# hi-paris/Prosody-Control-French-TTS

Measured on AMD Instinct MI355X. Metric: audio-seconds/sec prosody+align throughput, 16 kHz French, higher is better.
Workload: dtype fp16-resid16 (MFMA legs) + f64 (F0 / LUFS)

## Files before the change

prosody-control-french-tts_amd/csrc/pce_align.hip:

```cpp
#include "pce_internal.h"
#include <vector>

namespace {

constexpr int DTW_MAXN = 1024;

__global__ __launch_bounds__(DTW_MAXN) void k_dtw(const double *__restrict__ x, int64_t x_stride, int ld, const int *__restrict__ n_rows,
                                                 const int *__restrict__ n_cols, int N_max, int M_max, unsigned char *__restrict__ trace,
                                                 int *__restrict__ path_i, int *__restrict__ path_j, int *__restrict__ path_len)
{
    __shared__ float diag[3][DTW_MAXN + 1];
    const int b = blockIdx.x, t = threadIdx.x;
    const int N = n_rows ? n_rows[b] : N_max, M = n_cols ? n_cols[b] : M_max;
    if (N <= 0 || M <= 0) { if (t == 0) path_len[b] = 0; return; }
    const double *xb = x + (size_t)b * (size_t)x_stride;
    unsigned char *tr = trace + (size_t)b * (size_t)(N_max + 1) * (size_t)(M_max + 1);
    const float INF = __builtin_huge_valf();
    for (int r = t; r <= N; r += blockDim.x) { diag[0][r] = INF; diag[1][r] = INF; diag[2][r] = INF; }
    __syncthreads();
    if (t == 0) diag[0][0] = 0.0f;
    __syncthreads();
    const int r = t + 1;
    for (int D = 2; D <= N + M; D++) {
        float *cur = diag[D % 3]; const float *p1 = diag[(D - 1) % 3], *p2 = diag[(D - 2) % 3];
        const int c = D - r;
        if (t < N && c >= 1 && c <= M) {
            const float c0 = p2[r - 1], c1 = p1[r - 1], c2 = p1[r];
            float cm; unsigned char tt;
            if (c0 < c1 && c0 < c2) { cm = c0; tt = 0; }
            else if (c1 < c0 && c1 < c2) { cm = c1; tt = 1; }
            else { cm = c2; tt = 2; }
            cur[r] = (float)(xb[(size_t)(r - 1) * ld + (c - 1)] + (double)cm);
            tr[(size_t)r * (M + 1) + c] = tt;
        } else if (t < N) {
            cur[r] = INF;
        }
        if (t == 0) cur[0] = INF;
        __syncthreads();
    }
    __threadfence_block();
    if (t == 0) {
        int i = N, j = M, n = 0;
        int *pi = path_i + (size_t)b * (N_max + M_max), *pj = path_j + (size_t)b * (N_max + M_max);
        while (i > 0 || j > 0) {
            pi[n] = i - 1; pj[n] = j - 1; n++;
            const int tt = (i == 0) ? 2 : (j == 0) ? 1 : tr[(size_t)i * (M + 1) + j];
            if (tt == 0) { i--; j--; } else if (tt == 1) { i--; } else { j--; }
        }
        for (int a = 0, z = n - 1; a < z; a++, z--) {
            const int ti = pi[a], tj = pj[a]; pi[a] = pi[z]; pj[a] = pj[z]; pi[z] = ti; pj[z] = tj;
        }
        path_len[b] = n;
    }
}

__global__ __launch_bounds__(DTW_MAXN) void k_nw(const int *__restrict__ a_ids, const long long *__restrict__ a_off, const int *__restrict__ b_ids,
                                                const long long *__restrict__ b_off, int match, int mismatch, int gap,
                                                unsigned char *__restrict__ trace, const long long *__restrict__ tr_off,
                                                int *__restrict__ out_i, int *__restrict__ out_j, const long long *__restrict__ out_off,
                                                int *__restrict__ out_len, int *__restrict__ rows, const long long *__restrict__ rows_off)
{
    __shared__ int diag[3][DTW_MAXN + 1];
    const int b = blockIdx.x, t = threadIdx.x, S = (int)blockDim.x;
    const int N = (int)(a_off[b + 1] - a_off[b]), M = (int)(b_off[b + 1] - b_off[b]);
    const int *A = a_ids + a_off[b], *B = b_ids + b_off[b];
    unsigned char *tr = trace + tr_off[b];
    int *top = rows + rows_off[b], *bot = top + (M + 1);
    for (int r0 = 0; r0 < N; r0 += S) {
        const int R = min(S, N - r0), lr = t + 1, gr = r0 + lr;
        const bool first = r0 == 0, more = r0 + S < N;
        const int my_a = t < R ? A[gr - 1] : 0;
        if (t == 0) diag[0][0] = r0 * gap;
        int tv = (t == 0 && M >= 1) ? (first ? gap : top[1]) : 0;
        __syncthreads();
        for (int D = 1; D <= R + M; D++) {
            int *cur = diag[D % 3]; const int *p1 = diag[(D + 2) % 3], *p2 = diag[(D + 1) % 3];
            const int c = D - lr;
            if (t < R) {
                if (c >= 1 && c <= M) {
                    const int dg = p2[lr - 1] + (my_a == B[c - 1] ? match : mismatch), up = p1[lr - 1] + gap, lf = p1[lr] + gap;
                    int best = dg; unsigned char tt = 0;
                    if (up > best) { best = up; tt = 1; }
                    if (lf > best) { best = lf; tt = 2; }
                    cur[lr] = best;
                    tr[(size_t)gr * (M + 1) + c] = tt;
                    if (more && lr == R) bot[c] = best;
                } else if (c == 0) {
                    cur[lr] = gr * gap;
                }
            }
            if (t == 0 && D <= M) { cur[0] = tv; if (D + 1 <= M) tv = first ? (D + 1) * gap : top[D + 1]; }
            __syncthreads();
        }
        if (more) { __threadfence(); __syncthreads(); int *x = top; top = bot; bot = x; }
    }
    __threadfence_block();
    if (t == 0) {
        int i = N, j = M, n = 0;
        int *pi = out_i + out_off[b], *pj = out_j + out_off[b];
        while (i > 0 || j > 0) {
            const int tt = (i == 0) ? 2 : (j == 0) ? 1 : tr[(size_t)i * (M + 1) + j];
            if (tt == 0) { pi[n] = i - 1; pj[n] = j - 1; i--; j--; }
            else if (tt == 1) { pi[n] = i - 1; pj[n] = -1; i--; }
            else { pi[n] = -1; pj[n] = j - 1; j--; }
            n++;
        }
        for (int x = 0, z = n - 1; x < z; x++, z--) {
            const int ti = pi[x], tj = pj[x]; pi[x] = pi[z]; pj[x] = pj[z]; pi[z] = ti; pj[z] = tj;
        }
        out_len[b] = n;
    }
}

__global__ __launch_bounds__(256) void k_levenshtein(const unsigned *__restrict__ a_chars, const long long *__restrict__ a_off,
                                                     const unsigned *__restrict__ b_chars, const long long *__restrict__ b_off, int batch,
                                                     int *__restrict__ rows, const long long *__restrict__ rows_off, int *__restrict__ out)
{
    const int lane = threadIdx.x & 63, pair = blockIdx.x * 4 + __builtin_amdgcn_readfirstlane((int)(threadIdx.x >> 6));
    if (pair >= batch) return;
    int N = (int)(a_off[pair + 1] - a_off[pair]), M = (int)(b_off[pair + 1] - b_off[pair]);
    const unsigned *A = a_chars + a_off[pair], *B = b_chars + b_off[pair];
    if (N > M) { const unsigned *t = A; A = B; B = t; const int n = N; N = M; M = n; }
    if (N == 0) { if (lane == 0) out[pair] = M; return; }
    int *top = rows + rows_off[pair], *bot = top + (M + 1);
    const int n_stripes = (N + 63) >> 6;
    for (int s = 0; s < n_stripes; s++) {
        const int r0 = s << 6, R = min(64, N - r0), last = R - 1;
        const bool more = s + 1 < n_stripes;
        const unsigned my_a = lane < R ? A[r0 + lane] : 0u;
        int cur = r0 + lane + 1;
        int up = r0 + lane;
        unsigned bch = 0u;
        unsigned chB = lane < M ? B[lane] : 0u, nxB = 0u;
        int chT = s == 0 ? lane + 1 : (lane + 1 <= M ? top[lane + 1] : 0), nxT = 0;
        int botc = r0 + R;
        const int steps = M + R - 1;
        for (int t = 0; t < steps; t++) {
            const int k = t & 63;
            if (k == 0) {
                if (t) { chB = nxB; chT = nxT; }
                const int c1 = t + 64 + lane;
                nxB = c1 < M ? B[c1] : 0u;
                nxT = s == 0 ? c1 + 1 : (c1 + 1 <= M ? top[c1 + 1] : 0);
            }
            const unsigned b_in = (unsigned)__builtin_amdgcn_readlane((int)chB, k);
            const int top_in = __builtin_amdgcn_readlane(chT, k);
            const int upn_s = __builtin_amdgcn_update_dpp(0, cur, 0x138, 0xF, 0xF, true);
            const unsigned bch_s = (unsigned)__builtin_amdgcn_update_dpp(0, (int)bch, 0x138, 0xF, 0xF, true);
            const int upn = lane == 0 ? top_in : upn_s;
            bch = lane == 0 ? b_in : bch_s;
            const int c = t - lane + 1;
            if (lane < R && c >= 1 && c <= M) {
                const int sub = up + (my_a != bch ? 1 : 0), ins = upn + 1, del = cur + 1;
                cur = min(min(ins, del), sub);
                up = upn;
            }
            if (more) {
                const int cb = t - last + 1;
                if (cb >= 1) {
                    const int v = __builtin_amdgcn_readlane(cur, last);
                    if (lane == (cb & 63)) botc = v;
                    if ((cb & 63) == 63 || cb == M) {
                        const int base = cb & ~63;
                        if (lane <= (cb & 63)) bot[base + lane] = botc;
                    }
                }
            }
        }
        if (!more) { if (lane == last) out[pair] = cur; }
        else { __threadfence(); int *x = top; top = bot; bot = x; }
    }
}

}

int pce_dtw_launch(pce_ctx *c, const double *d_x, int64_t x_stride, int ld, const int *d_rows, const int *d_cols, int N_max, int M_max,
                   int batch, unsigned char *d_trace, int *d_pi, int *d_pj, int *d_pl)
{
    if (N_max > DTW_MAXN) return pce_fail(c, PCE_E_LIMIT, "DTW supports at most %d rows", DTW_MAXN);
    KernelTimer t(c, PCE_K_DTW);
    const int threads = ((N_max + 63) / 64) * 64;
    hipLaunchKernelGGL(k_dtw, dim3((unsigned)batch), dim3((unsigned)threads), 0, c->stream, d_x, x_stride, ld, d_rows, d_cols, N_max, M_max,
                       d_trace, d_pi, d_pj, d_pl);
    PCE_HIP(c, hipGetLastError());
    return PCE_OK;
}

extern "C" {

int pce_dtw(pce_ctx *c, const double *x, int32_t n_rows, int32_t n_cols, int32_t batch, int32_t *path_i, int32_t *path_j, int32_t *path_len)
{
    if (!c || !x || !path_i || !path_j || !path_len || n_rows <= 0 || n_cols <= 0 || batch <= 0) return PCE_E_INVALID;
    PCE_HIP(c, hipSetDevice(c->device));
    const size_t cells = (size_t)batch * n_rows * n_cols, pl = (size_t)batch * (size_t)(n_rows + n_cols);
    DevBuf dx, dtr, dpi, dpj, dpl;
    PCE_UPLOAD(c, dx, x, cells);
    PCE_HIP(c, dtr.reserve((size_t)batch * (size_t)(n_rows + 1) * (size_t)(n_cols + 1)));
    PCE_HIP(c, dpi.reserve(sizeof(int) * pl)); PCE_HIP(c, dpj.reserve(sizeof(int) * pl)); PCE_HIP(c, dpl.reserve(sizeof(int) * (size_t)batch));
    PCE_TRY(pce_dtw_launch(c, dx.as<double>(), (int64_t)n_rows * n_cols, n_cols, nullptr, nullptr, n_rows, n_cols, batch,
                           dtr.as<unsigned char>(), dpi.as<int>(), dpj.as<int>(), dpl.as<int>()));
    PCE_FETCH(c, path_i, dpi.p, pl);
    PCE_FETCH(c, path_j, dpj.p, pl);
    PCE_FETCH(c, path_len, dpl.p, (size_t)batch);
    PCE_HIP(c, hipStreamSynchronize(c->stream));
    pce_profile_collect(c);
    return PCE_OK;
}

int pce_nw_align(pce_ctx *c, const int32_t *a_ids, const int64_t *a_off, const int32_t *b_ids, const int64_t *b_off, int32_t batch,
                 int32_t match, int32_t mismatch, int32_t gap, int32_t *out_i, int32_t *out_j, int32_t *out_len)
{
    if (!c || !a_off || !b_off || !out_i || !out_j || !out_len || batch <= 0) return PCE_E_INVALID;
    PCE_HIP(c, hipSetDevice(c->device));
    std::vector<long long> tro((size_t)batch + 1, 0), oo((size_t)batch + 1, 0), rwo((size_t)batch + 1, 0);
    int max_rows = 0;
    for (int32_t b = 0; b < batch; b++) {
        const int64_t n = a_off[b + 1] - a_off[b], m = b_off[b + 1] - b_off[b];
        if (n < 0 || m < 0) return pce_fail(c, PCE_E_INVALID, "pce_nw_align: offsets of pair %d decrease", b);
        if (n > 0x3fffffff || m > 0x3fffffff) return pce_fail(c, PCE_E_LIMIT, "pce_nw_align: pair %d is longer than 2^30 tokens", b);
        tro[(size_t)b + 1] = tro[(size_t)b] + (n + 1) * (m + 1);
        rwo[(size_t)b + 1] = rwo[(size_t)b] + (n > DTW_MAXN ? 2 * (m + 1) : 0);
        oo[(size_t)b + 1] = oo[(size_t)b] + n + m;
        if (n > max_rows) max_rows = (int)n;
    }
    const size_t na = (size_t)a_off[batch], nb = (size_t)b_off[batch], no = (size_t)oo[(size_t)batch];
    if (a_off[0] != 0 || b_off[0] != 0) return pce_fail(c, PCE_E_INVALID, "pce_nw_align: offsets must start at 0");
    if ((na && !a_ids) || (nb && !b_ids)) return PCE_E_INVALID;
    DevBuf da, db, dao, dbo, dtr, dtro, doi, doj, doo, dol, drw, drwo;
    PCE_HIP(c, drw.reserve(sizeof(int) * ((size_t)rwo[(size_t)batch] + 1))); PCE_HIP(c, dtr.reserve((size_t)tro[(size_t)batch] + 1));
    PCE_HIP(c, doi.reserve(sizeof(int) * (no + 1))); PCE_HIP(c, doj.reserve(sizeof(int) * (no + 1))); PCE_HIP(c, dol.reserve(sizeof(int) * (size_t)batch));
    PCE_UPLOAD(c, da, a_ids, na, 1); PCE_UPLOAD(c, db, b_ids, nb, 1);
    PCE_UPLOAD(c, dao, a_off, (size_t)batch + 1); PCE_UPLOAD(c, dbo, b_off, (size_t)batch + 1);
    PCE_UPLOAD(c, dtro, tro); PCE_UPLOAD(c, doo, oo); PCE_UPLOAD(c, drwo, rwo);
    int threads = 64; while (threads < max_rows && threads < DTW_MAXN) threads <<= 1;
    {
        KernelTimer t(c, PCE_K_NW);
        hipLaunchKernelGGL(k_nw, dim3((unsigned)batch), dim3((unsigned)threads), 0, c->stream, da.as<int>(), dao.as<long long>(), db.as<int>(),
                           dbo.as<long long>(), match, mismatch, gap, dtr.as<unsigned char>(), dtro.as<long long>(), doi.as<int>(), doj.as<int>(),
                           doo.as<long long>(), dol.as<int>(), drw.as<int>(), drwo.as<long long>());
    }
    PCE_HIP(c, hipGetLastError());
    if (no) {
        PCE_FETCH(c, out_i, doi.p, no);
        PCE_FETCH(c, out_j, doj.p, no);
    }
    PCE_FETCH(c, out_len, dol.p, (size_t)batch);
    PCE_HIP(c, hipStreamSynchronize(c->stream));
    pce_profile_collect(c);
    return PCE_OK;
}

int pce_levenshtein(pce_ctx *c, const uint32_t *a_chars, const int64_t *a_off, const uint32_t *b_chars, const int64_t *b_off, int32_t batch,
                    int32_t *out_dist)
{
    if (!c || !a_off || !b_off || !out_dist || batch <= 0) return PCE_E_INVALID;
    PCE_HIP(c, hipSetDevice(c->device));
    if (a_off[0] != 0 || b_off[0] != 0) return pce_fail(c, PCE_E_INVALID, "pce_levenshtein: offsets must start at 0");
    std::vector<long long> ro((size_t)batch + 1, 0);
    for (int32_t b = 0; b < batch; b++) {
        const int64_t n = a_off[b + 1] - a_off[b], m = b_off[b + 1] - b_off[b];
        if (n < 0 || m < 0) return pce_fail(c, PCE_E_INVALID, "pce_levenshtein: offsets of pair %d decrease", b);
        if (n > 0x3fffffff || m > 0x3fffffff) return pce_fail(c, PCE_E_LIMIT, "pce_levenshtein: pair %d is longer than 2^30 characters", b);
        const int64_t shorter = n < m ? n : m, longer = n < m ? m : n;
        ro[(size_t)b + 1] = ro[(size_t)b] + (shorter > 64 ? 2 * (longer + 1) : 0);
    }
    const size_t na = (size_t)a_off[batch], nb = (size_t)b_off[batch];
    if ((na && !a_chars) || (nb && !b_chars)) return PCE_E_INVALID;
    DevBuf da, db, dao, dbo, dro, drows, dout;
    PCE_HIP(c, drows.reserve(sizeof(int) * ((size_t)ro[(size_t)batch] + 1))); PCE_HIP(c, dout.reserve(sizeof(int) * (size_t)batch));
    PCE_UPLOAD(c, da, a_chars, na, 1); PCE_UPLOAD(c, db, b_chars, nb, 1);
    PCE_UPLOAD(c, dao, a_off, (size_t)batch + 1); PCE_UPLOAD(c, dbo, b_off, (size_t)batch + 1); PCE_UPLOAD(c, dro, ro);
    {
        KernelTimer t(c, PCE_K_LEVENSHTEIN);
        hipLaunchKernelGGL(k_levenshtein, dim3((unsigned)((batch + 3) / 4)), dim3(256), 0, c->stream, da.as<unsigned>(), dao.as<long long>(),
                           db.as<unsigned>(), dbo.as<long long>(), batch, drows.as<int>(), dro.as<long long>(), dout.as<int>());
    }
    PCE_HIP(c, hipGetLastError());
    PCE_FETCH(c, out_dist, dout.p, (size_t)batch);
    PCE_HIP(c, hipStreamSynchronize(c->stream));
    pce_profile_collect(c);
    return PCE_OK;
}

}
```

prosody-control-french-tts_amd/csrc/pce_attention.inc:

```
constexpr int AT_QB = 128;

struct AttnArgs {
    const op_t *q; int64_t q_ld;
    const op_t *k; int64_t k_ld;
    const op_t *vt; int64_t vt_clip; int vt_sp;
    const int *q_row0, *q_len, *k_row0, *k_len;
    op_t *out; int64_t out_ld;
    int causal;
    int *fell_back;
};

template <bool EXACT, bool NT>
__device__ __forceinline__ bool attn_block16(const AttnArgs &A, op_t *smem, int bx, int head, int clip)
{
    constexpr int NS = 3, DPW = 4;
    const int tid = threadIdx.x, lane = tid & 63, wv = __builtin_amdgcn_readfirstlane(tid >> 6);
    const int n16 = lane & 15, g = lane >> 4;
    const int Sq = A.q_len[clip], Sk = A.k_len[clip];
    const int q0 = bx * AT_QB + wv * 32;
    const op_t *qbase = A.q + (int64_t)A.q_row0[clip] * A.q_ld + head * 64;
    const op_t *kbase = A.k + (int64_t)A.k_row0[clip] * A.k_ld + head * 64;
    const op_t *vtbase = A.vt + (int64_t)clip * A.vt_clip + (int64_t)head * 64 * A.vt_sp;
    const int kld = (int)A.k_ld, vsp = A.vt_sp;
    const __amdgpu_buffer_rsrc_t rsK = __builtin_amdgcn_make_buffer_rsrc(const_cast<op_t *>(kbase), 0, ((Sk - 1) * kld + 64) * 2, 0x00020000);
    const __amdgpu_buffer_rsrc_t rsV = __builtin_amdgcn_make_buffer_rsrc(const_cast<op_t *>(vtbase), 0, 64 * vsp * 2, 0x00020000);
    int voffK[2], voffV[2];
#pragma unroll
    for (int i = 0; i < 2; i++) {
        const int row = (wv + 4 * i) * 8 + (lane >> 3), c8 = swz_chunk(row, lane & 7) * 8;
        const int kb = row >> 4, rho = row & 15;
        const int key = 32 * (kb >> 1) + 8 * (rho >> 2) + 4 * (kb & 1) + (rho & 3);
        voffK[i] = (key * kld + c8) * 2; voffV[i] = (row * vsp + c8) * 2;
    }
    auto stage = [&](int t) {
        op_t *sK = smem + (t % NS) * (2 * 64 * 64), *sV = sK + 64 * 64;
        const int key0 = t * 64;
#pragma unroll
        for (int i = 0; i < 2; i++) {
            __builtin_amdgcn_raw_ptr_buffer_load_lds(rsK, (__attribute__((address_space(3))) void *)(sK + (wv + 4 * i) * 8 * 64), 16, voffK[i], key0 * kld * 2, 0, NT ? 3 : 0);
            __builtin_amdgcn_raw_ptr_buffer_load_lds(rsV, (__attribute__((address_space(3))) void *)(sV + (wv + 4 * i) * 8 * 64), 16, voffV[i], key0 * 2, 0, NT ? 3 : 0);
        }
    };
    const f32x4 z4 = {0.f, 0.f, 0.f, 0.f};
    opx8 qf[2][2];
    int my_q[2];
#pragma unroll
    for (int qb = 0; qb < 2; qb++) {
        my_q[qb] = q0 + 16 * qb + n16;
        int qr = my_q[qb]; if (qr >= Sq) qr = Sq - 1;
        const op_t *qp = qbase + (int64_t)qr * A.q_ld;
#pragma unroll
        for (int ks = 0; ks < 2; ks++) qf[qb][ks] = *reinterpret_cast<const opx8 *>(qp + 32 * ks + 8 * g);
    }
    opx8 ones;
#pragma unroll
    for (int j = 0; j < 8; j++) ones[j] = (op_t)(n16 == 0 ? 1.0f : 0.0f);
    f32x4 o[4][2], osum[2];
#pragma unroll
    for (int db = 0; db < 4; db++) { o[db][0] = z4; o[db][1] = z4; }
    osum[0] = z4; osum[1] = z4;
    float m_run[2] = {-1e30f, -1e30f}, l_run[2] = {0.f, 0.f};
    const float sl2 = 0.125f * 1.4426950408889634f;
    int k_need = Sk;
    if (A.causal) k_need = min(Sk, bx * AT_QB + AT_QB);
    const int nt = (k_need + 63) / 64;
    int kaddr[4][2], vaddr[4][2];
#pragma unroll
    for (int b4 = 0; b4 < 4; b4++)
#pragma unroll
        for (int ks = 0; ks < 2; ks++) {
            const int row = 16 * b4 + n16;
            kaddr[b4][ks] = row * 64 + swz_chunk(row, 4 * ks + g) * 8;
            vaddr[b4][ks] = 64 * 64 + row * 64 + swz_chunk(row, 4 * ks + g) * 8;
        }
    stage(0);
    if (nt > 1) stage(1);
    for (int kt = 0; kt < nt; kt++) {
        if (kt + 1 < nt) __builtin_amdgcn_s_waitcnt(0x0F70 | DPW); else __builtin_amdgcn_s_waitcnt(0x0F70 | 0);
        __builtin_amdgcn_s_barrier();
        if (kt + 2 < nt) stage(kt + 2);
        const op_t *sC = smem + (kt % NS) * (2 * 64 * 64);
        f32x4 sc[4][2];
#pragma unroll
        for (int kb = 0; kb < 4; kb++)
#pragma unroll
            for (int ks = 0; ks < 2; ks++) {
                const opx8 kf = *reinterpret_cast<const opx8 *>(&sC[kaddr[kb][ks]]);
#pragma unroll
                for (int qb = 0; qb < 2; qb++) sc[kb][qb] = mfma16(kf, qf[qb][ks], ks == 0 ? z4 : sc[kb][qb]);
            }
        if ((kt * 64 + 63 >= Sk) || (A.causal && kt * 64 + 63 > q0)) {
#pragma unroll
            for (int kb = 0; kb < 4; kb++)
#pragma unroll
                for (int i = 0; i < 4; i++) {
                    const int key = kt * 64 + 32 * (kb >> 1) + 8 * g + 4 * (kb & 1) + i;
#pragma unroll
                    for (int qb = 0; qb < 2; qb++) {
                        const bool vis = key < Sk && (!A.causal || key <= my_q[qb]);
                        sc[kb][qb][i] = vis ? sc[kb][qb][i] : -1e30f;
                    }
                }
        }
        if (EXACT || kt == 0) {
            float mx[2];
#pragma unroll
            for (int qb = 0; qb < 2; qb++) {
                float m = sc[0][qb][0];
#pragma unroll
                for (int kb = 0; kb < 4; kb++)
#pragma unroll
                    for (int i = 0; i < 4; i++) m = fmaxf(m, sc[kb][qb][i]);
                m = m > -1e29f ? m * sl2 : -1e30f;
                m = fmaxf(m, __shfl_xor(m, 16, 64));
                m = fmaxf(m, __shfl_xor(m, 32, 64));
                mx[qb] = fmaxf(m_run[qb], m);
            }
            if (__builtin_amdgcn_ballot_w64(mx[0] > m_run[0] || mx[1] > m_run[1]) != 0) {
#pragma unroll
                for (int qb = 0; qb < 2; qb++) {
                    const float corr = __builtin_amdgcn_exp2f(m_run[qb] - mx[qb]);
                    l_run[qb] *= corr;
#pragma unroll
                    for (int db = 0; db < 4; db++)
#pragma unroll
                        for (int i = 0; i < 4; i++) o[db][qb][i] *= corr;
                    m_run[qb] = mx[qb];
                }
            }
            if (!EXACT && std::is_same<op_t, _Float16>::value) { m_run[0] += 4.0f; m_run[1] += 4.0f; }
        }
        float rs[2] = {0.f, 0.f};
#pragma unroll
        for (int kb = 0; kb < 4; kb++)
#pragma unroll
            for (int qb = 0; qb < 2; qb++)
#pragma unroll
                for (int i = 0; i < 4; i++) {
                    const float pv = __builtin_amdgcn_exp2f(fmaf(sc[kb][qb][i], sl2, -m_run[qb]));
                    sc[kb][qb][i] = pv;
                    if (EXACT) rs[qb] += pv;
                }
        if (EXACT) {
#pragma unroll
            for (int qb = 0; qb < 2; qb++) {
                float sum = rs[qb];
                sum += __shfl_xor(sum, 16, 64);
                sum += __shfl_xor(sum, 32, 64);
                l_run[qb] += sum;
            }
        }
        opx8 vf[4][2];
#pragma unroll
        for (int db = 0; db < 4; db++)
#pragma unroll
            for (int s2 = 0; s2 < 2; s2++) vf[db][s2] = *reinterpret_cast<const opx8 *>(&sC[vaddr[db][s2]]);
#pragma unroll
        for (int s2 = 0; s2 < 2; s2++)
#pragma unroll
            for (int qb = 0; qb < 2; qb++) {
                opx8 pf;
#pragma unroll
                for (int i = 0; i < 4; i++) { pf[i] = (op_t)sc[2 * s2][qb][i]; pf[4 + i] = (op_t)sc[2 * s2 + 1][qb][i]; }
#pragma unroll
                for (int db = 0; db < 4; db++) o[db][qb] = mfma16(vf[db][s2], pf, o[db][qb]);
                if (!EXACT) osum[qb] = mfma16(ones, pf, osum[qb]);
            }
    }
    if (!EXACT) {
        l_run[0] = __shfl(osum[0][0], n16, 64);
        l_run[1] = __shfl(osum[1][0], n16, 64);
    }
    const bool ok = EXACT || (((l_run[0] > 0.f && l_run[0] < 1.0e30f) || my_q[0] >= Sq) && ((l_run[1] > 0.f && l_run[1] < 1.0e30f) || my_q[1] >= Sq));
    if (!EXACT && __syncthreads_or(!ok)) return false;
    typedef __attribute__((ext_vector_type(4))) op_t opx4;
#pragma unroll
    for (int qb = 0; qb < 2; qb++) {
        if (my_q[qb] >= Sq) continue;
        const float inv = 1.0f / l_run[qb];
        op_t *op = A.out + ((int64_t)A.q_row0[clip] + my_q[qb]) * A.out_ld + head * 64;
#pragma unroll
        for (int db = 0; db < 4; db++) {
            opx4 v4;
#pragma unroll
            for (int i = 0; i < 4; i++) v4[i] = (op_t)(o[db][qb][i] * inv);
            *reinterpret_cast<opx4 *>(op + 16 * db + 4 * g) = v4;
        }
    }
    return true;
}

template <bool NT>
__global__ __launch_bounds__(256, 3) void k_attention_lean16(AttnArgs A, int force_exact )
{
    __shared__ __attribute__((aligned(1024))) op_t smem[3 * 2 * 64 * 64];
    const unsigned nx = gridDim.x, ny = gridDim.y, total = nx * ny * gridDim.z;
    const unsigned lin = blockIdx.x + nx * (blockIdx.y + ny * blockIdx.z), xcd = lin & 7u, per = total >> 3, rem = total & 7u;
    const unsigned logical = xcd * per + (xcd < rem ? xcd : rem) + (lin >> 3);
    const int bx = (int)(logical % nx), head = (int)((logical / nx) % ny), clip = (int)(logical / (nx * ny));
    if (bx * AT_QB >= A.q_len[clip]) return;
    if (!force_exact && attn_block16<false, NT>(A, smem, bx, head, clip)) return;
    if (!force_exact && A.fell_back && threadIdx.x == 0) atomicAdd(A.fell_back, 1);
    __syncthreads();
    attn_block16<true, NT>(A, smem, bx, head, clip);
}

static void launch_attention(pce_ctx *c, dim3 grid, const AttnArgs &a, double flops = 0.0, int force_exact = 0 )
{
    KernelTimer kt(c, PCE_K_ATTENTION_LEAN, nullptr, flops);
    if (grid.x == 1) hipLaunchKernelGGL(k_attention_lean16<true>, grid, dim3(256), 0, c->stream, a, force_exact);
    else hipLaunchKernelGGL(k_attention_lean16<false>, grid, dim3(256), 0, c->stream, a, force_exact);
}
static void launch_attention_rows(pce_ctx *c, int n, int H, int q_rows, const op_t *q, int64_t q_ld, const op_t *k, int64_t k_ld, const op_t *vt, int vt_sp,
                                  const int *q_row0, const int *q_len, const int *k_row0, const int *k_len, op_t *out, int causal, double flops = 0.0)
{
    AttnArgs a{};
    a.q = q; a.q_ld = q_ld; a.k = k; a.k_ld = k_ld; a.vt = vt; a.vt_clip = (int64_t)H * 64 * vt_sp; a.vt_sp = vt_sp;
    a.q_row0 = q_row0; a.q_len = q_len; a.k_row0 = k_row0; a.k_len = k_len; a.out = out; a.out_ld = H * 64; a.causal = causal;
    launch_attention(c, dim3((unsigned)div_up(q_rows, AT_QB), (unsigned)H, (unsigned)n), a, flops);
}
```

Before: 21140.

## Keep small DTW traceback in LDS, prefetch cost rows, and skip empty attention query blocks

The DTW kernel now stores the traceback matrix in shared memory when it fits, prefetches cost values in register blocks of 16 diagonals, swaps diagonal pointers instead of using modulo indexing, and uses an LDS-only barrier. Backtracking writes the path in forward order in two passes instead of reversing it afterwards. The attention kernel specialises the inner tile on how many of the wave's two 16-row query blocks are valid, skipping MFMA and softmax work for out-of-range rows, and computes K/V LDS addresses from one base to lower register pressure. These changes add register use for the prefetch buffers and code-size growth from the template instantiations.

```diff
diff --git a/prosody-control-french-tts_amd/csrc/pce_align.hip b/prosody-control-french-tts_amd/csrc/pce_align.hip
--- a/prosody-control-french-tts_amd/csrc/pce_align.hip
+++ b/prosody-control-french-tts_amd/csrc/pce_align.hip
@@ -4,44 +4,87 @@
 namespace {
 
 constexpr int DTW_MAXN = 1024;
+constexpr int DTW_LDS_TRACE = 32 * 1024;
+constexpr int DTW_XB = 16;
+
+__device__ __forceinline__ void lds_barrier()
+{
+    __builtin_amdgcn_fence(__ATOMIC_RELEASE, "workgroup", "local");
+    __builtin_amdgcn_s_barrier();
+    __builtin_amdgcn_fence(__ATOMIC_ACQUIRE, "workgroup", "local");
+}
 
 __global__ __launch_bounds__(DTW_MAXN) void k_dtw(const double *__restrict__ x, int64_t x_stride, int ld, const int *__restrict__ n_rows,
                                                  const int *__restrict__ n_cols, int N_max, int M_max, unsigned char *__restrict__ trace,
                                                  int *__restrict__ path_i, int *__restrict__ path_j, int *__restrict__ path_len)
 {
     __shared__ float diag[3][DTW_MAXN + 1];
+    __shared__ unsigned char ltr[DTW_LDS_TRACE];
     const int b = blockIdx.x, t = threadIdx.x;
     const int N = n_rows ? n_rows[b] : N_max, M = n_cols ? n_cols[b] : M_max;
     if (N <= 0 || M <= 0) { if (t == 0) path_len[b] = 0; return; }
     const double *xb = x + (size_t)b * (size_t)x_stride;
     unsigned char *tr = trace + (size_t)b * (size_t)(N_max + 1) * (size_t)(M_max + 1);
+    const bool in_lds = (int64_t)(N + 1) * (int64_t)(M + 1) <= DTW_LDS_TRACE;
     const float INF = __builtin_huge_valf();
     for (int r = t; r <= N; r += blockDim.x) { diag[0][r] = INF; diag[1][r] = INF; diag[2][r] = INF; }
     __syncthreads();
     if (t == 0) diag[0][0] = 0.0f;
     __syncthreads();
     const int r = t + 1;
-    for (int D = 2; D <= N + M; D++) {
-        float *cur = diag[D % 3]; const float *p1 = diag[(D - 1) % 3], *p2 = diag[(D - 2) % 3];
-        const int c = D - r;
-        if (t < N && c >= 1 && c <= M) {
-            const float c0 = p2[r - 1], c1 = p1[r - 1], c2 = p1[r];
-            float cm; unsigned char tt;
-            if (c0 < c1 && c0 < c2) { cm = c0; tt = 0; }
-            else if (c1 < c0 && c1 < c2) { cm = c1; tt = 1; }
-            else { cm = c2; tt = 2; }
-            cur[r] = (float)(xb[(size_t)(r - 1) * ld + (c - 1)] + (double)cm);
-            tr[(size_t)r * (M + 1) + c] = tt;
-        } else if (t < N) {
-            cur[r] = INF;
-        }
-        if (t == 0) cur[0] = INF;
-        __syncthreads();
-    }
-    __threadfence_block();
+    const double *xrow = xb + (size_t)min(t, N - 1) * ld;
+    float *cur = diag[2], *p1 = diag[1], *p2 = diag[0];
+    auto fetch = [&](double (&dst)[DTW_XB], int D0) __attribute__((always_inline)) {
+#pragma unroll
+        for (int j = 0; j < DTW_XB; j++) dst[j] = xrow[min(max(D0 + j - r - 1, 0), M - 1)];
+    };
+    auto block = [&](const double (&xc)[DTW_XB], double (&xn)[DTW_XB], int D0) __attribute__((always_inline)) {
+        fetch(xn, D0 + DTW_XB);
+#pragma unroll
+        for (int j = 0; j < DTW_XB; j++) {
+            const int D = D0 + j;
+            if (D > N + M) break;
+            const int c = D - r;
+            if (t < N && c >= 1 && c <= M) {
+                const float c0 = p2[r - 1], c1 = p1[r - 1], c2 = p1[r];
+                float cm; unsigned char tt;
+                if (c0 < c1 && c0 < c2) { cm = c0; tt = 0; }
+                else if (c1 < c0 && c1 < c2) { cm = c1; tt = 1; }
+                else { cm = c2; tt = 2; }
+                cur[r] = (float)(xc[j] + (double)cm);
+                if (in_lds) ltr[r * (M + 1) + c] = tt; else tr[(size_t)r * (M + 1) + c] = tt;
+            } else if (t < N) {
+                cur[r] = INF;
+            }
+            if (t == 0) cur[0] = INF;
+            lds_barrier();
+            float *const old = p2; p2 = p1; p1 = cur; cur = old;
+        }
+    };
+    double xa[DTW_XB], xz[DTW_XB];
+    fetch(xa, 2);
+    for (int D0 = 2; D0 <= N + M; D0 += 2 * DTW_XB) {
+        block(xa, xz, D0);
+        block(xz, xa, D0 + DTW_XB);
+    }
+    __syncthreads();
     if (t == 0) {
+        int *pi = path_i + (size_t)b * (N_max + M_max), *pj = path_j + (size_t)b * (N_max + M_max);
+        if (in_lds) {
+            int n = 0;
+            for (int i = N, j = M; i > 0 || j > 0; n++) {
+                const int tt = (i == 0) ? 2 : (j == 0) ? 1 : ltr[i * (M + 1) + j];
+                if (tt == 0) { i--; j--; } else if (tt == 1) { i--; } else { j--; }
+            }
+            path_len[b] = n;
+            for (int i = N, j = M, k = n - 1; i > 0 || j > 0; k--) {
+                pi[k] = i - 1; pj[k] = j - 1;
+                const int tt = (i == 0) ? 2 : (j == 0) ? 1 : ltr[i * (M + 1) + j];
+                if (tt == 0) { i--; j--; } else if (tt == 1) { i--; } else { j--; }
+            }
+            return;
+        }
         int i = N, j = M, n = 0;
-        int *pi = path_i + (size_t)b * (N_max + M_max), *pj = path_j + (size_t)b * (N_max + M_max);
         while (i > 0 || j > 0) {
             pi[n] = i - 1; pj[n] = j - 1; n++;
             const int tt = (i == 0) ? 2 : (j == 0) ? 1 : tr[(size_t)i * (M + 1) + j];
diff --git a/prosody-control-french-tts_amd/csrc/pce_attention.inc b/prosody-control-french-tts_amd/csrc/pce_attention.inc
--- a/prosody-control-french-tts_amd/csrc/pce_attention.inc
+++ b/prosody-control-french-tts_amd/csrc/pce_attention.inc
@@ -64,30 +64,26 @@
     int k_need = Sk;
     if (A.causal) k_need = min(Sk, bx * AT_QB + AT_QB);
     const int nt = (k_need + 63) / 64;
-    int kaddr[4][2], vaddr[4][2];
-#pragma unroll
-    for (int b4 = 0; b4 < 4; b4++)
-#pragma unroll
-        for (int ks = 0; ks < 2; ks++) {
-            const int row = 16 * b4 + n16;
-            kaddr[b4][ks] = row * 64 + swz_chunk(row, 4 * ks + g) * 8;
-            vaddr[b4][ks] = 64 * 64 + row * 64 + swz_chunk(row, 4 * ks + g) * 8;
-        }
-    stage(0);
-    if (nt > 1) stage(1);
-    for (int kt = 0; kt < nt; kt++) {
-        if (kt + 1 < nt) __builtin_amdgcn_s_waitcnt(0x0F70 | DPW); else __builtin_amdgcn_s_waitcnt(0x0F70 | 0);
-        __builtin_amdgcn_s_barrier();
-        if (kt + 2 < nt) stage(kt + 2);
+    int faddr[2];
+#pragma unroll
+    for (int ks = 0; ks < 2; ks++) {
+        faddr[ks] = n16 * 64 + swz_chunk(n16, 4 * ks + g) * 8;
+        asm volatile("" : "+v"(faddr[ks]));
+    }
+    auto kaddr = [&](int b4, int ks) __attribute__((always_inline)) { return faddr[ks] + 16 * 64 * b4; };
+    auto vaddr = [&](int b4, int ks) __attribute__((always_inline)) { return faddr[ks] + 64 * 64 + 16 * 64 * b4; };
+    const int nq = __builtin_amdgcn_readfirstlane(q0 >= Sq ? 0 : q0 + 16 >= Sq ? 1 : 2);
+    auto tile = [&](auto nq_c, int kt) __attribute__((always_inline)) {
+        constexpr int NQ = decltype(nq_c)::value;
         const op_t *sC = smem + (kt % NS) * (2 * 64 * 64);
         f32x4 sc[4][2];
 #pragma unroll
         for (int kb = 0; kb < 4; kb++)
 #pragma unroll
             for (int ks = 0; ks < 2; ks++) {
-                const opx8 kf = *reinterpret_cast<const opx8 *>(&sC[kaddr[kb][ks]]);
-#pragma unroll
-                for (int qb = 0; qb < 2; qb++) sc[kb][qb] = mfma16(kf, qf[qb][ks], ks == 0 ? z4 : sc[kb][qb]);
+                const opx8 kf = *reinterpret_cast<const opx8 *>(&sC[kaddr(kb, ks)]);
+#pragma unroll
+                for (int qb = 0; qb < NQ; qb++) sc[kb][qb] = mfma16(kf, qf[qb][ks], ks == 0 ? z4 : sc[kb][qb]);
             }
         if ((kt * 64 + 63 >= Sk) || (A.causal && kt * 64 + 63 > q0)) {
 #pragma unroll
@@ -96,7 +92,7 @@
                 for (int i = 0; i < 4; i++) {
                     const int key = kt * 64 + 32 * (kb >> 1) + 8 * g + 4 * (kb & 1) + i;
 #pragma unroll
-                    for (int qb = 0; qb < 2; qb++) {
+                    for (int qb = 0; qb < NQ; qb++) {
                         const bool vis = key < Sk && (!A.causal || key <= my_q[qb]);
                         sc[kb][qb][i] = vis ? sc[kb][qb][i] : -1e30f;
                     }
@@ -105,7 +101,7 @@
         if (EXACT || kt == 0) {
             float mx[2];
 #pragma unroll
-            for (int qb = 0; qb < 2; qb++) {
+            for (int qb = 0; qb < NQ; qb++) {
                 float m = sc[0][qb][0];
 #pragma unroll
                 for (int kb = 0; kb < 4; kb++)
@@ -116,9 +112,9 @@
                 m = fmaxf(m, __shfl_xor(m, 32, 64));
                 mx[qb] = fmaxf(m_run[qb], m);
             }
-            if (__builtin_amdgcn_ballot_w64(mx[0] > m_run[0] || mx[1] > m_run[1]) != 0) {
-#pragma unroll
-                for (int qb = 0; qb < 2; qb++) {
+            if (__builtin_amdgcn_ballot_w64(mx[0] > m_run[0] || (NQ == 2 && mx[1] > m_run[1])) != 0) {
+#pragma unroll
+                for (int qb = 0; qb < NQ; qb++) {
                     const float corr = __builtin_amdgcn_exp2f(m_run[qb] - mx[qb]);
                     l_run[qb] *= corr;
 #pragma unroll
@@ -128,13 +124,13 @@
                     m_run[qb] = mx[qb];
                 }
             }
-            if (!EXACT && std::is_same<op_t, _Float16>::value) { m_run[0] += 4.0f; m_run[1] += 4.0f; }
+            if (!EXACT && std::is_same<op_t, _Float16>::value) { m_run[0] += 4.0f; if (NQ == 2) m_run[1] += 4.0f; }
         }
         float rs[2] = {0.f, 0.f};
 #pragma unroll
         for (int kb = 0; kb < 4; kb++)
 #pragma unroll
-            for (int qb = 0; qb < 2; qb++)
+            for (int qb = 0; qb < NQ; qb++)
 #pragma unroll
                 for (int i = 0; i < 4; i++) {
                     const float pv = __builtin_amdgcn_exp2f(fmaf(sc[kb][qb][i], sl2, -m_run[qb]));
@@ -143,7 +139,7 @@
                 }
         if (EXACT) {
 #pragma unroll
-            for (int qb = 0; qb < 2; qb++) {
+            for (int qb = 0; qb < NQ; qb++) {
                 float sum = rs[qb];
                 sum += __shfl_xor(sum, 16, 64);
                 sum += __shfl_xor(sum, 32, 64);
@@ -154,11 +150,11 @@
 #pragma unroll
         for (int db = 0; db < 4; db++)
 #pragma unroll
-            for (int s2 = 0; s2 < 2; s2++) vf[db][s2] = *reinterpret_cast<const opx8 *>(&sC[vaddr[db][s2]]);
+            for (int s2 = 0; s2 < 2; s2++) vf[db][s2] = *reinterpret_cast<const opx8 *>(&sC[vaddr(db, s2)]);
 #pragma unroll
         for (int s2 = 0; s2 < 2; s2++)
 #pragma unroll
-            for (int qb = 0; qb < 2; qb++) {
+            for (int qb = 0; qb < NQ; qb++) {
                 opx8 pf;
 #pragma unroll
                 for (int i = 0; i < 4; i++) { pf[i] = (op_t)sc[2 * s2][qb][i]; pf[4 + i] = (op_t)sc[2 * s2 + 1][qb][i]; }
@@ -166,7 +162,20 @@
                 for (int db = 0; db < 4; db++) o[db][qb] = mfma16(vf[db][s2], pf, o[db][qb]);
                 if (!EXACT) osum[qb] = mfma16(ones, pf, osum[qb]);
             }
-    }
+    };
+    auto tiles = [&](auto nq_c) __attribute__((always_inline)) {
+        for (int kt = 0; kt < nt; kt++) {
+            if (kt + 1 < nt) __builtin_amdgcn_s_waitcnt(0x0F70 | DPW); else __builtin_amdgcn_s_waitcnt(0x0F70 | 0);
+            __builtin_amdgcn_s_barrier();
+            if (kt + 2 < nt) stage(kt + 2);
+            if (decltype(nq_c)::value > 0) tile(nq_c, kt);
+        }
+    };
+    stage(0);
+    if (nt > 1) stage(1);
+    if (nq == 2) tiles(std::integral_constant<int, 2>{});
+    else if (nq == 1) tiles(std::integral_constant<int, 1>{});
+    else tiles(std::integral_constant<int, 0>{});
     if (!EXACT) {
         l_run[0] = __shfl(osum[0][0], n16, 64);
         l_run[1] = __shfl(osum[1][0], n16, 64);
```

After: 21310 (median of 6 runs). No clear change (+0.8%).
